# qutech/filter_functions

Hardware: AMD Instinct MI355X
Metric: filter-function elements/sec (n_seg*n_omega*n_nops*d^2) at d=4 (higher is better)
Workload: dtype f64

## Files before the change

### filter_functions_amd/csrc/ctrl_pq.hip

```cpp
#include <algorithm>
#include <cstdlib>

#include "ffk_internal.h"
#include "ffk_mfma_util.h"

namespace ffk {
namespace {

constexpr int kPqProducers = 4;
constexpr int kPqSets = 2;
constexpr int kPqConsumers = 16/kPqSets;
constexpr int kPqRing = 8;
#ifndef FFK_PC_SPIN_LIMIT
#define FFK_PC_SPIN_LIMIT (1 << 21)
#endif
constexpr int kPqSpinLimit = FFK_PC_SPIN_LIMIT;

__device__ __forceinline__ void pq_report_fault(int* fault, int code) {
    if (fault != nullptr && (threadIdx.x & 63) == 0)
        __hip_atomic_store(fault, code, __ATOMIC_RELAXED, __HIP_MEMORY_SCOPE_SYSTEM);
}

typedef double double2_t __attribute__((ext_vector_type(2)));
typedef double double4_t __attribute__((ext_vector_type(4)));
typedef double double8_t __attribute__((ext_vector_type(8)));
typedef int int4_t __attribute__((ext_vector_type(4)));
typedef __attribute__((address_space(3))) int lds_int_t;

template <int NC>
struct PqConsumer;
#include "ctrl_pq_consumer.inc"

constexpr int kPqQ = 0, kPqPsi = 1024, kPqW = 1152;
constexpr int kPqRow = seg_stride(4);
__host__ __device__ constexpr int pq_tile_doubles(int nc) { return kPqW + nc*128 + 32; }
__host__ __device__ constexpr int pq_lds_bytes_for(int nc) {
    return (kPqRing*pq_tile_doubles(nc) + kPqProducers*kPqRow)*8 + 3*kPqRing*4;
}

__device__ __forceinline__ int lds_peek(const int* flag) {
    return __builtin_amdgcn_readfirstlane(*(const volatile lds_int_t*)(flag));
}

template <int NC, bool PRE>
__global__ __launch_bounds__((kPqProducers + kPqConsumers)*64, 3) void ctrl_accumulate_pq_kernel(
    const double* __restrict__ omega, int W, const double* __restrict__ segtab,
    const cplx* __restrict__ ops, int G, int A, int chunk_len, cplx* __restrict__ Ypart,
    const cplx* __restrict__ wfold, int alpha_base, int alpha_end, int* __restrict__ fault_word) {
    constexpr int D = 4, DD = 16, S = kPqRow, TILE = pq_tile_doubles(NC);
    constexpr int TOP = kPqW + NC*128;
    static_assert(PqConsumer<NC>::kTileBytes == TILE*8, "tools/gen_pq_consumer.py and pq_tile_doubles() disagree");
    extern __shared__ __attribute__((aligned(16))) unsigned char lds_raw[];
    double* ring = reinterpret_cast<double*>(lds_raw);
    double* rows = ring + kPqRing*TILE;
    int* ready = reinterpret_cast<int*>(rows + kPqProducers*S);
    int* done = ready + kPqRing;

    const int lane = threadIdx.x & 63;
    const int wave = __builtin_amdgcn_readfirstlane(threadIdx.x >> 6);
    const int alpha0 = alpha_base + blockIdx.y*NC;
    const int n_alpha = min(NC, alpha_end - alpha0);
    const int g0 = blockIdx.z*chunk_len;
    const int g1 = min(G, g0 + chunk_len);
    const int n_it = max(0, g1 - g0);
    int spin_limit = kPqSpinLimit;

    if (threadIdx.x < 3*kPqRing) *(volatile lds_int_t*)(ready + threadIdx.x) = 0;
    __syncthreads();

    if (wave < kPqProducers) {
        __builtin_amdgcn_s_setprio(0);
        const int iw = blockIdx.x*64 + lane;
        double om = omega[iw < W ? iw : W - 1];
        asm volatile("" : "+v"(om));
        const int n_ops = (1 + n_alpha)*DD;
        double* row = rows + wave*S;
        struct Staged {
            cplx o;
            double r0, r1;
        };
        auto request = [&](int it) __attribute__((always_inline)) -> Staged {
            const int g = g0 + it;
            const cplx* src = ops + static_cast<size_t>(g)*(1 + A)*DD;
            const double* st = segtab + static_cast<size_t>(g)*S;
            Staged t;
            if constexpr (PRE) {
                t.o = cplx{0.0, 0.0};
                t.r0 = st[lane];
                t.r1 = st[64 + (lane & (S - 64 - 1))];
            } else {
                t.o = lane < n_ops ? src[lane < DD ? lane : lane + alpha0*DD] : cplx{0.0, 0.0};
                t.r0 = st[lane];
                t.r1 = lane < S - 64 ? st[64 + lane] : 0.0;
            }
            return t;
        };
        auto wait_slot = [&](int slot, int gen) __attribute__((always_inline)) {
            if (gen > 0) {
                int spin = 0;
                for (; spin < spin_limit; ++spin) {
                    if (lds_peek(done + slot) >= gen*kPqConsumers) break;
                    __builtin_amdgcn_s_sleep(2);
                }
                if (spin == spin_limit && spin_limit != 0) {
                    pq_report_fault(fault_word, kFaultPcProducerWait);
                    spin_limit = 0;
                }
                asm volatile("" ::: "memory");
            }
        };
        Staged cur = {};
        if (wave < n_it) cur = request(wave);
        for (int it = wave; it < n_it; it += kPqProducers) {
            const int slot = it & (kPqRing - 1);
            const int gen = it/kPqRing;
            double* buf = ring + slot*TILE;
            row[lane] = cur.r0;
            if (lane < S - 64) row[64 + lane] = cur.r1;
            const cplx o = cur.o;
            if constexpr (PRE) {
                wait_slot(slot, gen);
                const size_t gw = (static_cast<size_t>(g0 + it)*A + alpha0)*64;
#pragma unroll
                for (int a = 0; a < NC; ++a)
                    if (a < n_alpha) lds_dma16(wfold + gw + a*64 + lane, buf + kPqW + a*128);
                if (lane < DD) lds_dma16(ops + static_cast<size_t>(g0 + it)*(1 + A)*DD + lane, buf + TOP);
            }
            if (it + kPqProducers < n_it) cur = request(it + kPqProducers);
            const double* st = row;
            const double2_t sbcb = *reinterpret_cast<const double2_t*>(st + seg_rec(lane >> 2) + 1);
            const double2_t head = *reinterpret_cast<const double2_t*>(st);
            const double sb = sbcb.x, cb = sbcb.y;
            const double dtg = head.x;
            cplx ph;
            sincos_pi<false>(om*head.y, &ph.im, &ph.re);
            double sa, ca;
            sincos_pi<false>(0.5*(om*dtg), &sa, &ca);
            const PhasedFrequency pf = phased_frequency(om, dtg, ph, sa, ca);
            double q[DD];
            auto batch = [&](int e0, int e1) __attribute__((always_inline)) {
                double4_t rec[DD];
#pragma unroll
                for (int e = 0; e < DD; ++e) {
                    if (e < e0 || e >= e1 || (e != 0 && e/D == e%D)) continue;
                    rec[e] = *reinterpret_cast<const double4_t*>(st + seg_rec(e));
                }
                asm volatile("" ::: "memory");
                double xmin = pf.thr;
#pragma unroll
                for (int e = 0; e < DD; ++e) {
                    if (e < e0 || e >= e1 || (e != 0 && e/D == e%D)) continue;
                    const double x = om + rec[e].x;
                    q[e] = fma(pf.sa2, rec[e].z, pf.ca2*rec[e].y)*rcp_fast(x);
                    asm("v_min_f64 %0, |%1|, %0" : "+v"(xmin) : "v"(x));
                }
                if (xmin < pf.thr) {
#pragma unroll
                    for (int e = 0; e < DD; ++e) {
                        if (e < e0 || e >= e1 || (e != 0 && e/D == e%D)) continue;
                        if (fabs(om + rec[e].x) < pf.thr) q[e] = phased_q(pf, rec[e].x, rec[e].y, rec[e].z);
                    }
                }
            };
            batch(0, 8);
            batch(8, 16);
            q[5] = q[0];
            q[10] = q[0];
            q[15] = q[0];
            if constexpr (!PRE) wait_slot(slot, gen);
#pragma unroll
            for (int h = 0; h < 2; ++h)
#pragma unroll
                for (int m = 0; m < D; ++m) {
                    const double2_t v = {q[m*D + 2*h], q[m*D + 2*h + 1]};
                    *reinterpret_cast<double2_t*>(buf + kPqQ + h*512 + lane*8 + (((m ^ (lane >> 2)) & 3) << 1)) = v;
                }
            {
                const double2_t v = {pf.pr, pf.pi};
                *reinterpret_cast<double2_t*>(buf + kPqPsi + lane*2) = v;
            }
            if constexpr (!PRE) {
                const int src_t = lane & (DD - 1);
                const cplx tv = {__shfl(o.re, src_t, 64), __shfl(o.im, src_t, 64)};
                const cplx et = cmul(cplx{cb, sb}, tv);
                const int wslot = ((lane >> 2) & 3)*16 + (lane >> 4)*4 + (lane & 3);
#pragma unroll
                for (int a = 0; a < NC; ++a) {
                    const int src_b = DD + a*DD + (lane >> 2);
                    const cplx bv = {__shfl(o.re, src_b, 64), __shfl(o.im, src_b, 64)};
                    const cplx w = cmul(bv, et);
                    const double2_t v = {w.re, w.im};
                    *reinterpret_cast<double2_t*>(buf + kPqW + a*128 + wslot*2) = v;
                }
            }
            if constexpr (PRE) {
                if (it + kPqProducers < n_it) asm volatile("s_waitcnt vmcnt(2)" ::: "memory");
                else lds_dma_wait();
            } else if (lane < DD) {
                const double2_t v = {o.re, o.im};
                *reinterpret_cast<double2_t*>(buf + TOP + lane*2) = v;
            }
            asm volatile("s_waitcnt lgkmcnt(0)" ::: "memory");
#ifdef FFK_PC_FAULT_INJECT
            if (it < 2*kPqProducers)
#endif
            if (lane == 0) *(volatile lds_int_t*)(ready + slot) = it + 1;
        }
        return;
    }

    const int octant = wave - kPqProducers;
    const int m = lane >> 4, f = (lane >> 2) & 3, j = lane & 3;
    const int mj = m*4 + j;
    const int wf = octant*4*kPqSets + f;
    const int o_w = kPqW + mj*2;
    const int o_p = kPqPsi + wf*2;
    const int o_q0 = kPqQ + wf*8 + ((m ^ ((kPqSets*octant) & 3)) << 1);
    const int o_q1 = (o_q0 ^ 2) + 32;
    double P[6*NC];
#pragma unroll
    for (int k = 0; k < 6*NC; ++k) P[k] = 0.0;
    if (n_it > 0) {
        int spin = 0;
        for (; spin < spin_limit; ++spin) {
            if (lds_peek(ready) >= 1) break;
            __builtin_amdgcn_s_sleep(1);
        }
        if (spin == spin_limit) {
            pq_report_fault(fault_word, kFaultPcConsumerWait);
            spin_limit = 0;
        }
        asm volatile("" ::: "memory");
        const unsigned ring_b = static_cast<unsigned>(reinterpret_cast<uintptr_t>(ring));
        const unsigned flags_b = static_cast<unsigned>(reinterpret_cast<uintptr_t>(ready));
        const int fault_code = PqConsumer<NC>::run(ring_b + o_w*8, ring_b + o_q0*8, ring_b + o_q1*8, ring_b + o_p*8, n_it,
                                                   spin_limit, flags_b, octant, P);
        if (fault_code != 0) pq_report_fault(fault_word, fault_code);
    }
#pragma unroll
    for (int a = 0; a < NC; ++a) {
        const int alpha = alpha0 + a;
        if (alpha >= alpha_end) break;
        cplx* out = Ypart + ((static_cast<size_t>(blockIdx.z)*A + alpha)*DD + mj)*W;
#pragma unroll
        for (int s = 0; s < kPqSets; ++s) {
            const int iw = blockIdx.x*64 + wf + s*4;
            const double p1 = P[3*(kPqSets*a + s)], p2 = P[3*(kPqSets*a + s) + 1], p3 = P[3*(kPqSets*a + s) + 2];
            if (iw < W) out[iw] = cplx{p1 - p2, p3 - (p1 + p2)};
        }
    }
}

template <int NC, bool PRE>
hipError_t launch_pq_as(const double* omega, int W, const double* segtab, const cplx* ops, int G, int A,
                        int chunks, int chunk_len, cplx* Ypart, const cplx* wfold, int alpha_base, int alpha_end,
                        int* fault_word, hipStream_t stream) {
    const int lds = pq_lds_bytes_for(NC);
    auto kern = ctrl_accumulate_pq_kernel<NC, PRE>;
    hipError_t err = hipFuncSetAttribute(reinterpret_cast<const void*>(kern),
                                         hipFuncAttributeMaxDynamicSharedMemorySize, lds);
    if (err != hipSuccess) return err;
    const int n = alpha_end - alpha_base;
    const dim3 grid((W + 63)/64, (n + NC - 1)/NC, chunks);
    hipLaunchKernelGGL(kern, grid, dim3((kPqProducers + kPqConsumers)*64), lds, stream, omega, W, segtab,
                       ops, G, A, chunk_len, Ypart, wfold, alpha_base, alpha_end, fault_word);
    return hipGetLastError();
}

template <int NC>
hipError_t launch_pq(const double* omega, int W, const double* segtab, const cplx* ops, int G, int A,
                     int chunks, int chunk_len, cplx* Ypart, const cplx* wfold, int alpha_base, int alpha_end,
                     int* fault_word, hipStream_t stream) {
    return wfold != nullptr ? launch_pq_as<NC, true>(omega, W, segtab, ops, G, A, chunks, chunk_len, Ypart, wfold,
                                                     alpha_base, alpha_end, fault_word, stream)
                            : launch_pq_as<NC, false>(omega, W, segtab, ops, G, A, chunks, chunk_len, Ypart, nullptr,
                                                      alpha_base, alpha_end, fault_word, stream);
}

}

int pq_accumulate_lds_bytes(int nc) { return pq_lds_bytes_for(nc); }
int pq_accumulate_waves(int) { return kPqProducers + kPqConsumers; }
bool pq_accumulate_supported(int d, int A) { return d == 4 && A >= 1; }

PqGroups pq_accumulate_groups(int A) {
    if (A <= 0) return {0, 0, 0};
    if (A == 1) return {0, 0, 1};
    switch (A % 3) {
        case 0: return {A/3, 0, 0};
        case 1: return {(A - 4)/3, 2, 0};
        default: return {(A - 2)/3, 1, 0};
// ... 29 lines not shown
```

### filter_functions_amd/csrc/ffk_math.h

```cpp
#pragma once

#include <hip/hip_runtime.h>

#include <cmath>

#define FFK_HD __host__ __device__ __forceinline__

namespace ffk {

struct cplx {
    double re, im;
};

FFK_HD cplx cmul(cplx a, cplx b) {
    return {fma(a.re, b.re, -(a.im*b.im)), fma(a.re, b.im, a.im*b.re)};
}
FFK_HD void cmac(cplx& acc, cplx a, cplx b) {
    acc.re = fma(a.re, b.re, acc.re);
    acc.re = fma(-a.im, b.im, acc.re);
    acc.im = fma(a.re, b.im, acc.im);
    acc.im = fma(a.im, b.re, acc.im);
}
FFK_HD void cmac_conj(cplx& acc, cplx a, cplx b) {
    acc.re = fma(a.re, b.re, acc.re);
    acc.re = fma(a.im, b.im, acc.re);
    acc.im = fma(a.re, b.im, acc.im);
    acc.im = fma(-a.im, b.re, acc.im);
}

template <unsigned long long BITS>
FFK_HD double pinned_bits() {
#if defined(__HIP_DEVICE_COMPILE__)
    unsigned lo, hi;
    asm volatile("v_mov_b32 %0, %1" : "=v"(lo) : "n"(static_cast<unsigned>(BITS & 0xffffffffull)));
    asm volatile("v_mov_b32 %0, %1" : "=v"(hi) : "n"(static_cast<unsigned>(BITS >> 32)));
    return __hiloint2double(static_cast<int>(hi), static_cast<int>(lo));
#else
    return __builtin_bit_cast(double, BITS);
#endif
}
#define FFK_PIN(c) (PIN ? pinned_bits<__builtin_bit_cast(unsigned long long, static_cast<double>(c))>() : (c))

template <bool PIN = false>
FFK_HD void sincos_reduced(double r, double* s, double* c) {
    const double z = r*r;
    double ps = fma(z, FFK_PIN(1.58969099521155010221e-10), FFK_PIN(-2.50507602534068634195e-08));
    ps = fma(z, ps, FFK_PIN(2.75573137070700676789e-06));
    ps = fma(z, ps, FFK_PIN(-1.98412698298579493134e-04));
    ps = fma(z, ps, FFK_PIN(8.33333333332248946124e-03));
    ps = fma(z, ps, FFK_PIN(-1.66666666666666324348e-01));
    *s = fma(r*z, ps, r);
    double pc = fma(z, FFK_PIN(-1.13596475577881948265e-11), FFK_PIN(2.08757232129817482790e-09));
    pc = fma(z, pc, FFK_PIN(-2.75573143513906633035e-07));
    pc = fma(z, pc, FFK_PIN(2.48015872894767294178e-05));
    pc = fma(z, pc, FFK_PIN(-1.38888888888741095749e-03));
    pc = fma(z, pc, FFK_PIN(4.16666666666666019037e-02));
    const double hz = 0.5*z;
    const double w = 1.0 - hz;
    *c = w + (((1.0 - w) - hz) + z*z*pc);
}

template <bool PIN = false>
FFK_HD void sincos_small(double r, double* s, double* c) {
    const double z = r*r;
    double ps = fma(z, FFK_PIN(2.75573137070700676789e-06), FFK_PIN(-1.98412698298579493134e-04));
    ps = fma(z, ps, FFK_PIN(8.33333333332248946124e-03));
    ps = fma(z, ps, FFK_PIN(-1.66666666666666324348e-01));
    *s = fma(r*z, ps, r);
    double pc = fma(z, FFK_PIN(2.48015872894767294178e-05), FFK_PIN(-1.38888888888741095749e-03));
    pc = fma(z, pc, FFK_PIN(4.16666666666666019037e-02));
    const double hz = 0.5*z;
    const double w = 1.0 - hz;
    *c = w + (((1.0 - w) - hz) + z*z*pc);
}

FFK_HD unsigned low_word(double t) {
#if defined(__HIP_DEVICE_COMPILE__)
    return static_cast<unsigned>(__double2loint(t));
#else
    unsigned long long bits;
    __builtin_memcpy(&bits, &t, sizeof bits);
    return static_cast<unsigned>(bits);
#endif
}

template <bool PIN = false>
FFK_HD void sincos_pi(double x, double* s, double* c) {
    const double kMagic = FFK_PIN(6755399441055744.0);
    const double t = fma(x, FFK_PIN(6.36619772367581382433e-01), kMagic);
    const unsigned q = low_word(t);
    const double k = t - kMagic;
    double r = fma(-k, FFK_PIN(1.57079632679489655800e+00), x);
    r = fma(-k, FFK_PIN(6.12323399573676603587e-17), r);
    r = fma(-k, FFK_PIN(-1.49738490485916983294e-33), r);
    double sr, cr;
    sincos_reduced<PIN>(r, &sr, &cr);
    const double s0 = (q & 1u) ? cr : sr;
    const double c0 = (q & 1u) ? sr : cr;
    *s = (q & 2u) ? -s0 : s0;
    *c = ((q + 1u) & 2u) ? -c0 : c0;
}

#undef FFK_PIN

FFK_HD double rcp(double x) {
#if defined(__HIP_DEVICE_COMPILE__)
    double y = __builtin_amdgcn_rcp(x);
    double e = fma(-x, y, 1.0);
    y = fma(y, e, y);
    e = fma(-x, y, 1.0);
    y = fma(y, e, y);
    return y;
#else
    return 1.0/x;
#endif
}

FFK_HD double rcp_fast(double x) {
#if defined(__HIP_DEVICE_COMPILE__)
    double y = __builtin_amdgcn_rcp(x);
    const double e = fma(-x, y, 1.0);
    return fma(y, e, y);
#else
    return 1.0/x;
#endif
}

FFK_HD double rsqrt(double x) {
#if defined(__HIP_DEVICE_COMPILE__)
    double y = __builtin_amdgcn_rsq(x);
    double e = fma(-x*y, y, 1.0);
    y = fma(y, 0.5*e, y);
    e = fma(-x*y, y, 1.0);
    y = fma(y, 0.5*e, y);
    return y;
#else
    return 1.0/sqrt(x);
#endif
}

FFK_HD cplx first_order_integral(double omega, double dE, double dt) {
    const double x = omega + dE;
    const double y = x*dt;
    double s, c;
    sincos_pi(0.5*y, &s, &c);
    const double q = 2.0*s*rcp(x);
    cplx out = {q*c, q*s};
    if (x == 0.0) {
        out.re = dt;
        out.im = 0.0;
    }
    return out;
}

FFK_HD cplx first_order_integral_aa(double omega, double dE, double dt, double sa, double ca,
                                    double sb, double cb) {
    const double x = omega + dE;
    const double h = 0.5*(x*dt);
    double s = fma(sa, cb, ca*sb);
    double c = fma(ca, cb, -(sa*sb));
    if (fabs(h) < 0.03125) sincos_small<true>(h, &s, &c);
    const double q = 2.0*s*rcp_fast(x);
    cplx out = {q*c, q*s};
    if (x == 0.0) {
        out.re = dt;
        out.im = 0.0;
    }
    return out;
}

struct PhasedFrequency {
    double om, dt, thr;
    double pr, pi;
    double sa2, ca2;
};
FFK_HD PhasedFrequency phased_frequency(double om, double dt, cplx ph, double sa, double ca) {
    PhasedFrequency f;
    f.om = om;
    f.dt = dt;
    f.thr = dt > 0.0 ? 0.0625*rcp(dt) : __builtin_huge_val();
    f.pr = fma(ph.re, ca, -(ph.im*sa));
    f.pi = fma(ph.re, sa, ph.im*ca);
    f.sa2 = sa + sa;
    f.ca2 = ca + ca;
    return f;
}
FFK_HD double phased_q(const PhasedFrequency& f, double dE, double sb, double cb) {
    const double x = f.om + dE;
    double q;
    if (fabs(x) < f.thr) {
        double s, c;
        sincos_small<true>(0.5*(x*f.dt), &s, &c);
        q = x == 0.0 ? f.dt : 2.0*s*rcp_fast(x);
    } else {
        q = fma(f.sa2, cb, f.ca2*sb)*rcp_fast(x);
    }
    return q;
}
FFK_HD cplx phased_integral_aa(const PhasedFrequency& f, double dE, double sb, double cb) {
    const double er = fma(f.pr, cb, -(f.pi*sb));
    const double ei = fma(f.pr, sb, f.pi*cb);
    const double q = phased_q(f, dE, sb, cb);
    return {q*er, q*ei};
}

FFK_HD cplx cexp(double x) {
    cplx out;
    sincos_pi(x, &out.im, &out.re);
    return out;
}

}
```

### filter_functions_amd/csrc/post.hip

```cpp
#include <algorithm>

#include <cstdlib>

#include "ffk_internal.h"

namespace ffk {
namespace {

__global__ void reduce_chunks_kernel(const cplx* __restrict__ Ypart, int chunks, size_t slab,
                                     cplx* __restrict__ Bt) {
    const size_t e = static_cast<size_t>(blockIdx.x)*blockDim.x + threadIdx.x;
    if (e >= slab) return;
    cplx acc = Ypart[e];
    for (int c = 1; c < chunks; ++c) {
        const cplx v = Ypart[static_cast<size_t>(c)*slab + e];
        acc.re += v.re;
        acc.im += v.im;
    }
    Bt[e] = acc;
}

__global__ __launch_bounds__(64) void basis_compact_kernel(const cplx* __restrict__ basis, int d,
                                                           int* __restrict__ nnz,
                                                           int* __restrict__ rows,
// ... 198 lines not shown
    const int a0 = ba*TB, b0 = bb*TB;
    cplx acc[TB][TB];
#pragma unroll
    for (int i = 0; i < TB; ++i)
#pragma unroll
        for (int j = 0; j < TB; ++j) acc[i][j] = {0.0, 0.0};
    for (int k = 0; k < N; ++k) {
        cplx ra[TB], rb[TB];
#pragma unroll
        for (int i = 0; i < TB; ++i) {
            const int a = min(a0 + i, A - 1), b = min(b0 + i, A - 1);
            ra[i] = R[(static_cast<size_t>(a)*N + k)*W + w];
            rb[i] = R[(static_cast<size_t>(b)*N + k)*W + w];
        }
#pragma unroll
        for (int i = 0; i < TB; ++i)
#pragma unroll
            for (int j = 0; j < TB; ++j) cmac_conj(acc[i][j], ra[i], rb[j]);
    }
#pragma unroll
    for (int i = 0; i < TB; ++i)
#pragma unroll
        for (int j = 0; j < TB; ++j) {
            const int a = a0 + i, b = b0 + j;
            if (a >= A || b >= A || a > b) continue;
            cplx v = acc[i][j];
            if (a == b) v.im = 0.0;
            F[(static_cast<size_t>(a)*A + b)*W + w] = v;
            if (a != b) F[(static_cast<size_t>(b)*A + a)*W + w] = {v.re, -v.im};
        }
    }
}

template <int TB, int NT>
__global__ __launch_bounds__(NT*64) void ff_fidelity_lds_kernel(const cplx* __restrict__ R, int A, int N, int W,
                                                             int kc, cplx* __restrict__ F) {
    extern __shared__ __attribute__((aligned(16))) unsigned char ffl_raw[];
    cplx* buf = reinterpret_cast<cplx*>(ffl_raw);
    const int tid = threadIdx.x, lane = tid & 63;
    const int wave = __builtin_amdgcn_readfirstlane(tid >> 6);
    const int nwaves = blockDim.x >> 6;
    const int nb = (A + TB - 1)/TB;
    int ba = 0, rem = wave;
    while (rem >= nb - ba) {
        rem -= nb - ba;
        ++ba;
    }
    const int bb = ba + rem;
    const int a0 = ba*TB, b0 = bb*TB;
    const int w0 = blockIdx.x*64;
    const int w = w0 + lane;
    const int wc = min(w, W - 1);
    const int rows = kc*A;
    constexpr int kMaxRows = 12;
    const cplx* src[kMaxRows];
    int dst[kMaxRows];
#pragma unroll
    for (int r = 0; r < kMaxRows; ++r) {
        const int row = min(wave + r*nwaves, rows - 1);
        src[r] = R + (static_cast<size_t>(row % A)*N + row / A)*W + wc;
        dst[r] = row*64 + lane;
    }
    cplx acc[TB][TB];
#pragma unroll
    for (int i = 0; i < TB; ++i)
#pragma unroll
        for (int j = 0; j < TB; ++j) acc[i][j] = {0.0, 0.0};
#pragma unroll
    for (int r = 0; r < kMaxRows; ++r) buf[dst[r]] = src[r][0];
    __syncthreads();
    int b = 0;
    for (int k0 = 0; k0 < N; k0 += kc) {
        cplx staged[kMaxRows];
        const size_t knext = static_cast<size_t>(min(k0 + kc, N - kc < 0 ? 0 : N - kc))*W;
#pragma unroll
        for (int r = 0; r < kMaxRows; ++r) staged[r] = src[r][knext];
        const int kn = min(kc, N - k0);
        for (int kk = 0; kk < kn; ++kk) {
            const cplx* rowp = buf + (static_cast<size_t>(b)*rows + kk*A)*64 + lane;
            cplx ra[TB], rb[TB];
#pragma unroll
            for (int i = 0; i < TB; ++i) {
                ra[i] = rowp[min(a0 + i, A - 1)*64];
                rb[i] = rowp[min(b0 + i, A - 1)*64];
            }
#pragma unroll
            for (int i = 0; i < TB; ++i)
#pragma unroll
                for (int j = 0; j < TB; ++j) cmac_conj(acc[i][j], ra[i], rb[j]);
        }
#pragma unroll
        for (int r = 0; r < kMaxRows; ++r) buf[static_cast<size_t>(b ^ 1)*rows*64 + dst[r]] = staged[r];
        __syncthreads();
        b ^= 1;
    }
    if (w >= W) return;
#pragma unroll
    for (int i = 0; i < TB; ++i)
#pragma unroll
        for (int j = 0; j < TB; ++j) {
            const int a = a0 + i, bq = b0 + j;
            if (a >= A || bq >= A || a > bq) continue;
            cplx v = acc[i][j];
            if (a == bq) v.im = 0.0;
            F[(static_cast<size_t>(a)*A + bq)*W + w] = v;
            if (a != bq) F[(static_cast<size_t>(bq)*A + a)*W + w] = {v.re, -v.im};
        }
}

__global__ __launch_bounds__(128) void ff_weighted_kernel(const cplx* __restrict__ R, int A, int N,
                                                          int W, const cplx* __restrict__ M,
                                                          double scale, cplx* __restrict__ F) {
    const int w = blockIdx.x*blockDim.x + threadIdx.x;
    if (w >= W) return;
    for (long long pair = blockIdx.y; pair < static_cast<long long>(A)*A; pair += gridDim.y) {
        const int a = static_cast<int>(pair / A), b = static_cast<int>(pair % A);
        const cplx* ra = R + static_cast<size_t>(a)*N*W + w;
        const cplx* rb = R + static_cast<size_t>(b)*N*W + w;
        cplx acc = {0.0, 0.0};
        for (int k = 0; k < N; ++k) {
            cplx u = {0.0, 0.0};
            for (int l = 0; l < N; ++l) cmac(u, M[k*N + l], rb[static_cast<size_t>(l)*W]);
            cmac_conj(acc, ra[static_cast<size_t>(k)*W], u);
        }
        F[(static_cast<size_t>(a)*A + b)*W + w] = {scale*acc.re, scale*acc.im};
    }
}

__global__ void ff_generalized_kernel(const cplx* __restrict__ R, int A, int N, int W,
                                      cplx* __restrict__ F) {
    const int w = blockIdx.x*blockDim.x + threadIdx.x;
    if (w >= W) return;
    for (long long ab = blockIdx.z; ab < static_cast<long long>(A)*A; ab += gridDim.z) {
        const int a = static_cast<int>(ab / A), b = static_cast<int>(ab % A);
        for (long long kl = blockIdx.y; kl < static_cast<long long>(N)*N; kl += gridDim.y) {
            const int k = static_cast<int>(kl / N), l = static_cast<int>(kl % N);
            const cplx x = R[(static_cast<size_t>(a)*N + k)*W + w];
            const cplx y = R[(static_cast<size_t>(b)*N + l)*W + w];
            const double rr = x.re*y.re;
            const double ii = x.im*y.im;
            const double ri = x.re*y.im;
            const double ir = x.im*y.re;
            cplx v;
            v.re = rr + ii;
            v.im = ri - ir;
            F[((((static_cast<size_t>(a)*A + b)*N + k)*N + l))*W + w] = v;
        }
    }
}

constexpr int kInfidSlots = 1024, kInfidThreads = 256;
constexpr int kInfidPer = kInfidSlots/kInfidThreads;

template <int J0, int JN, typename LoadF, typename LoadS>
__device__ __forceinline__ void infid_batch(int base, int W, const double* __restrict__ omega, LoadF Fat, LoadS Sat,
                                            double (&acc)[kInfidPer], double* red = nullptr) {
    const int lane = threadIdx.x & 63;
    cplx f[kInfidPer], sp[kInfidPer];
    double om[kInfidPer];
#pragma unroll
    for (int j = J0; j < J0 + JN; ++j) {
        const int w = base + static_cast<int>(threadIdx.x) + kInfidThreads*j;
        const int wc = w < W ? w : W - 1;
        f[j] = Fat(wc);
        sp[j] = Sat(wc);
        om[j] = omega[wc];
    }
#pragma unroll
    for (int j = J0; j < J0 + JN; ++j) {
        const int w = base + static_cast<int>(threadIdx.x) + kInfidThreads*j;
        const double i0 = f[j].re*sp[j].re - f[j].im*sp[j].im;
        double i1 = __shfl_down(i0, 1, 64), o1 = __shfl_down(om[j], 1, 64);
        if (lane == 63 && w + 1 < W) {
            const cplx f1 = Fat(w + 1), s1 = Sat(w + 1);
            i1 = f1.re*s1.re - f1.im*s1.im;
            o1 = omega[w + 1];
        }
        if (w < W - 1) {
            if (red != nullptr) red[threadIdx.x + kInfidThreads*j] += (i1 + i0)*(o1 - om[j]);
            else acc[j] += (i1 + i0)*(o1 - om[j]);
        }
    }
}

template <bool FROM_REGISTERS = true>
__device__ __forceinline__ void infid_finish(double* red, const double (&acc)[kInfidPer], int d, double* out) {
    static_assert(kInfidPer == 4 && kInfidThreads == 256, "the tree below is written for 4 slots per thread, 4 wavefronts");
    double sl[kInfidPer];
#pragma unroll
    for (int j = 0; j < kInfidPer; ++j) sl[j] = FROM_REGISTERS ? acc[j] : red[threadIdx.x + kInfidThreads*j];
    double x = (sl[0] + sl[2]) + (sl[1] + sl[3]);
    __syncthreads();
    red[threadIdx.x] = x;
    __syncthreads();
    if (threadIdx.x < 128) red[threadIdx.x] = x = x + red[threadIdx.x + 128];
    __syncthreads();
    if (threadIdx.x < 64) {
        x = x + red[threadIdx.x + 64];
#pragma unroll
        for (int off = 32; off > 0; off >>= 1) x = x + __shfl_down(x, off, 64);
        if (threadIdx.x == 0) *out = (x/2.0)/(2.0*3.141592653589793*d);
    }
}

template <bool SHARDED>
__device__ __forceinline__ void infid_element(const cplx* __restrict__ F, int A, int W,
                                              const cplx* __restrict__ S, int s_ndim,
                                              const double* __restrict__ omega,
                                              const int32_t* __restrict__ idx, int n_idx,
                                              int d, int shard_width,
                                              double* __restrict__ infid, const int p) {
    __shared__ double red[kInfidSlots];
    __builtin_amdgcn_s_setprio(3);
    int ia, ib;
    const cplx* Sp;
    if (s_ndim == 3) {
        ia = idx[p / n_idx];
        ib = idx[p % n_idx];
        Sp = S + static_cast<size_t>(p)*W;
    } else {
        ia = ib = idx[p];
        Sp = S + (s_ndim == 2 ? static_cast<size_t>(p)*W : 0);
    }
    const cplx* Fp = F + (static_cast<size_t>(ia)*A + ib)*(SHARDED ? shard_width : W);
    auto Fat = [&](int w) -> cplx {
        if (SHARDED) {
            const int r = w / shard_width, wl = w - r*shard_width;
            return Fp[static_cast<size_t>(r)*A*A*shard_width + wl];
        }
        return Fp[w];
    };
    auto Sat = [&](int w) -> cplx { return Sp[w]; };
    double acc[kInfidPer];
#pragma unroll
    for (int j = 0; j < kInfidPer; ++j) red[threadIdx.x + kInfidThreads*j] = 0.0;
    for (int base = 0; base < W - 1; base += kInfidSlots) {
        infid_batch<0, kInfidPer>(base, W, omega, Fat, Sat, acc, red);
        asm volatile("" ::: "memory");
    }
    infid_finish<false>(red, acc, d, infid + p);
}

template <bool SHARDED>
__global__ __launch_bounds__(kInfidThreads) void infid_kernel(const cplx* __restrict__ F, int A, int W,
                                                              const cplx* __restrict__ S, int s_ndim,
                                                              const double* __restrict__ omega,
                                                              const int32_t* __restrict__ idx, int n_idx,
                                                              int d, int shard_width,
                                                              double* __restrict__ infid) {
    infid_element<SHARDED>(F, A, W, S, s_ndim, omega, idx, n_idx, d, shard_width, infid, blockIdx.x);
}

__global__ __launch_bounds__(kInfidThreads) void infid_pulses_kernel(const cplx* __restrict__ F, int A, int W,
                                                                     const cplx* __restrict__ S, int s_ndim,
                                                                     const double* __restrict__ omega,
                                                                     const int32_t* __restrict__ idx, int n_idx,
                                                                     int d, int nout, double* __restrict__ infid) {
    const size_t q = blockIdx.y;
    infid_element<false>(F + q*A*A*W, A, W, S, s_ndim, omega, idx, n_idx, d, 0, infid + q*nout, blockIdx.x);
}

constexpr int kInfidStage = 4096;
__global__ __launch_bounds__(kInfidThreads) void infid_host_spectrum_kernel(
    const cplx* __restrict__ F, int A, int W, const cplx* __restrict__ S, int s_ndim,
    const double* __restrict__ omega, const int32_t* __restrict__ idx, int n_idx, int d,
    double* __restrict__ infid) {
    __shared__ double red[kInfidSlots];
    extern __shared__ __attribute__((aligned(16))) unsigned char stage_raw[];
    cplx* sl = reinterpret_cast<cplx*>(stage_raw);
    const int p = blockIdx.x;
    int ia, ib;
    const cplx* Sp;
    if (s_ndim == 3) {
        ia = idx[p / n_idx];
        ib = idx[p % n_idx];
        Sp = S + static_cast<size_t>(p)*W;
    } else {
        ia = ib = idx[p];
        Sp = S + (s_ndim == 2 ? static_cast<size_t>(p)*W : 0);
    }
    const cplx* Fp = F + (static_cast<size_t>(ia)*A + ib)*W;
    constexpr int kLoads = kInfidStage/kInfidThreads + 1;
    double acc[kInfidPer];
#pragma unroll
    for (int j = 0; j < kInfidPer; ++j) acc[j] = 0.0;
    for (int s0 = 0; s0 < W - 1; s0 += kInfidStage) {
        const int n = min(kInfidStage + 1, W - s0);
        cplx v[kLoads];
#pragma unroll
        for (int k = 0; k < kLoads; ++k) {
            const int i = threadIdx.x + kInfidThreads*k;
            v[k] = i < n ? Sp[s0 + i] : cplx{0.0, 0.0};
        }
#pragma unroll
        for (int k = 0; k < kLoads; ++k) {
            const int i = threadIdx.x + kInfidThreads*k;
            if (i < n) sl[i] = v[k];
        }
        __syncthreads();
        auto Fat = [&](int w) -> cplx { return Fp[w]; };
        auto Sat = [&](int w) -> cplx { return sl[w - s0]; };
        const int bend = min(W - 1, s0 + kInfidStage);
        for (int base = s0; base < bend; base += kInfidSlots) infid_batch<0, kInfidPer>(base, W, omega, Fat, Sat, acc);
        __syncthreads();
    }
    infid_finish(red, acc, d, infid + p);
}

}

hipError_t launch_reduce_chunks(const cplx* Ypart, int chunks, size_t slab, cplx* Bt,
                                hipStream_t stream) {
    const int block = 256;
    hipLaunchKernelGGL(reduce_chunks_kernel, dim3(static_cast<unsigned>((slab + block - 1)/block)),
                       dim3(block), 0, stream, Ypart, chunks, slab, Bt);
    return hipGetLastError();
}

size_t expand_workspace_bytes(int N, int d) {
    const size_t dd = static_cast<size_t>(d)*d;
    return align_up(sizeof(int)*N) + align_up(sizeof(int)*N*dd) + align_up(sizeof(cplx)*N*dd);
}

namespace {
struct CompactWs {
    int* nnz;
    int* rows;
    cplx* vals;
};
CompactWs slice_compact_ws(void* ws, int N, int d) {
    const size_t dd = static_cast<size_t>(d)*d;
    unsigned char* p = static_cast<unsigned char*>(ws);
    CompactWs out;
    out.nnz = reinterpret_cast<int*>(p);
    p += align_up(sizeof(int)*N);
    out.rows = reinterpret_cast<int*>(p);
    p += align_up(sizeof(int)*N*dd);
    out.vals = reinterpret_cast<cplx*>(p);
    return out;
}
}

hipError_t launch_reduce_and_compact(const cplx* Ypart, int chunks, size_t slab, cplx* Bt,
                                     const cplx* basis, int N, int d, void* ws, hipStream_t stream) {
    const CompactWs c = slice_compact_ws(ws, N, d);
    const int block = 256;
    const int nred = static_cast<int>((slab + block - 1)/block);
    hipLaunchKernelGGL(reduce_compact_kernel, dim3(nred + N), dim3(block), 0, stream, Ypart, chunks,
                       slab, Bt, nred, basis, d, c.nnz, c.rows, c.vals);
    return hipGetLastError();
}

void expand_workspace_slices(void* ws, int N, int d, int** nnz, int** rows, cplx** vals) {
    const CompactWs cw = slice_compact_ws(ws, N, d);
    *nnz = cw.nnz;
    *rows = cw.rows;
    *vals = cw.vals;
}

__global__ __launch_bounds__(64) void expand_chunks_kernel(const cplx* __restrict__ Ypart, int chunks,
                                                           size_t slab, const int* __restrict__ nnz,
                                                           const int* __restrict__ rows,
                                                           const cplx* __restrict__ vals, int N,
                                                           int dd, int W, cplx* __restrict__ R) {
    const int w = blockIdx.x*64 + threadIdx.x;
    const int a = blockIdx.y, k = blockIdx.z;
    if (w >= W) return;
    const cplx* b = Ypart + static_cast<size_t>(a)*dd*W + w;
    const int n = nnz[k];
    const int* rk = rows + static_cast<size_t>(k)*dd;
    const cplx* vk = vals + static_cast<size_t>(k)*dd;
    auto summed = [&](int e) {
        cplx acc = b[static_cast<size_t>(e)*W];
        for (int z = 1; z < chunks; ++z) {
            const cplx v = b[z*slab + static_cast<size_t>(e)*W];
            acc.re += v.re;
            acc.im += v.im;
        }
        return acc;
    };
    cplx acc0 = {0.0, 0.0}, acc1 = {0.0, 0.0};
    int q = 0;
    for (; q + 1 < n; q += 2) {
        cmac(acc0, vk[q], summed(rk[q]));
        cmac(acc1, vk[q + 1], summed(rk[q + 1]));
    }
    if (q < n) cmac(acc0, vk[q], summed(rk[q]));
    R[(static_cast<size_t>(a)*N + k)*W + w] = {acc0.re + acc1.re, acc0.im + acc1.im};
}

__device__ __forceinline__ void expand_ff_tile(const cplx* __restrict__ Ypart, int chunks, size_t slab,
                                               const int* __restrict__ nnz, const int* __restrict__ rows,
                                               const cplx* __restrict__ vals, int N, int dd, int W, int A,
                                               int kt, cplx* __restrict__ R, cplx* __restrict__ F) {
    extern __shared__ __attribute__((aligned(16))) unsigned char lds_raw[];
    cplx* rl = reinterpret_cast<cplx*>(lds_raw);
    __builtin_amdgcn_s_setprio(3);
    cplx* ys = rl + static_cast<size_t>(A)*N*16;
    const int wl = threadIdx.x & 15;
    const int kl = (threadIdx.x >> 4) % kt, al = (threadIdx.x >> 4) / kt;
    const int at = (blockDim.x >> 4) / kt;
    const int w = blockIdx.x*16 + wl;
    const int wc = w < W ? w : W - 1;
    for (int idx = threadIdx.x >> 4; idx < A*dd; idx += blockDim.x >> 4) {
        const cplx* b = Ypart + static_cast<size_t>(idx)*W + wc;
        cplx acc = b[0];
        for (int z = 1; z < chunks; ++z) {
            const cplx v = b[z*slab];
            acc.re += v.re;
            acc.im += v.im;
        }
        ys[static_cast<size_t>(idx)*16 + wl] = acc;
    }
    __syncthreads();
    for (int a = al; a < A; a += at) {
        const cplx* ya = ys + static_cast<size_t>(a)*dd*16 + wl;
        for (int k = kl; k < N; k += kt) {
            const int n = nnz[k];
            const int* rk = rows + static_cast<size_t>(k)*dd;
            const cplx* vk = vals + static_cast<size_t>(k)*dd;
            auto summed = [&](int e) { return ya[e*16]; };
            cplx acc0 = {0.0, 0.0}, acc1 = {0.0, 0.0};
            int q = 0;
            for (; q + 1 < n; q += 2) {
                cmac(acc0, vk[q], summed(rk[q]));
                cmac(acc1, vk[q + 1], summed(rk[q + 1]));
            }
            if (q < n) cmac(acc0, vk[q], summed(rk[q]));
            const cplx r = {acc0.re + acc1.re, acc0.im + acc1.im};
            rl[(static_cast<size_t>(a)*N + k)*16 + wl] = r;
            if (w < W) R[(static_cast<size_t>(a)*N + k)*W + w] = r;
        }
    }
    __syncthreads();
    if (w >= W) return;
    const int npairs = A*(A + 1)/2;
    const int lanes = blockDim.x >> 4;
    for (int p = threadIdx.x >> 4; p < npairs; p += lanes) {
        int a = 0, rem = p;
        while (rem >= A - a) {
            rem -= A - a;
            ++a;
        }
        const int b = a + rem;
        const cplx* ra = rl + static_cast<size_t>(a)*N*16 + wl;
        const cplx* rb = rl + static_cast<size_t>(b)*N*16 + wl;
        cplx acc = {0.0, 0.0};
        for (int k = 0; k < N; ++k) cmac_conj(acc, ra[k*16], rb[k*16]);
        if (a == b) acc.im = 0.0;
        F[(static_cast<size_t>(a)*A + b)*W + w] = acc;
        if (a != b) F[(static_cast<size_t>(b)*A + a)*W + w] = {acc.re, -acc.im};
    }
}

__global__ __launch_bounds__(256) void expand_ff_kernel(const cplx* __restrict__ Ypart, int chunks,
                                                         size_t slab, const int* __restrict__ nnz,
// ... 265 lines not shown
```

### filter_functions_amd/csrc/prep.hip

```cpp
#include "ffk_internal.h"

namespace ffk {
namespace {

template <int D>
__device__ void prologue_segment(const cplx (*V)[D], cplx (*Q)[D], cplx (*T)[D], cplx (*BV)[D],
                                 int g, int lane, const double* __restrict__ eigvals,
                                 const cplx* __restrict__ n_opers,
                                 const double* __restrict__ n_coeffs,
                                 const double* __restrict__ dt, const double* __restrict__ t, int G,
                                 int A, double* __restrict__ segtab, cplx* __restrict__ Tc,
                                 cplx* __restrict__ ops, cplx* __restrict__ n_opers_transformed,
                                 cplx* __restrict__ eigvecs_propagated, bool with_noise_ops = true,
                                 cplx* __restrict__ wfold = nullptr) {
    constexpr int S = seg_stride(D);
    double* st = segtab + static_cast<size_t>(g)*S;
    if (lane == 0) {
        st[0] = dt[g];
        st[1] = t[g];
    }
    cplx eb = {1.0, 0.0};
    for (int e = lane; e < D*D; e += 64) {
        const double dE = eigvals[static_cast<size_t>(g)*D + e / D] - eigvals[static_cast<size_t>(g)*D + e % D];
        double sb, cb;
        sincos_pi(0.5*(dE*dt[g]), &sb, &cb);
        st[seg_rec(e)] = dE;
        st[seg_rec(e) + 1] = sb;
        st[seg_rec(e) + 2] = cb;
        st[seg_rec(e) + 3] = 0.0;
        eb = {cb, sb};
    }
    if (lane < 2) st[2 + lane] = 0.0;
    for (int e = 4 + 4*D*D + lane; e < S; e += 64) st[e] = 0.0;

    for (int e = lane; e < D*D; e += 64) {
        const int m = e / D, j = e % D;
        cplx acc = {0.0, 0.0};
#pragma unroll
        for (int k = 0; k < D; ++k) cmac_conj(acc, V[k][m], Q[k][j]);
        T[m][j] = acc;
        Tc[static_cast<size_t>(g)*D*D + e] = {acc.re, -acc.im};
        ops[static_cast<size_t>(g)*(1 + A)*D*D + e] = acc;
        if (eigvecs_propagated)
            eigvecs_propagated[static_cast<size_t>(g)*D*D + j*D + m] = {acc.re, -acc.im};
    }
    __syncthreads();

    if (!with_noise_ops) return;
    const bool fold = D == 4 && wfold != nullptr;
    if (fold) {
        if (lane < D*D) Q[lane / D][lane % D] = eb;
        __syncthreads();
    }
    for (int a = 0; a < A; ++a) {
        const cplx* B = n_opers + static_cast<size_t>(a)*D*D;
        const double s = n_coeffs ? n_coeffs[static_cast<size_t>(a)*G + g] : 1.0;
        for (int e = lane; e < D*D; e += 64) {
            const int i = e / D, n = e % D;
            cplx acc = {0.0, 0.0};
#pragma unroll
            for (int k = 0; k < D; ++k) cmac(acc, B[i*D + k], V[k][n]);
            BV[i][n] = acc;
        }
        __syncthreads();
        cplx bbar = {0.0, 0.0};
        for (int e = lane; e < D*D; e += 64) {
            const int m = e / D, n = e % D;
            cplx acc = {0.0, 0.0};
#pragma unroll
            for (int k = 0; k < D; ++k) cmac_conj(acc, V[k][m], BV[k][n]);
            acc.re *= s;
            acc.im *= s;
            ops[(static_cast<size_t>(g)*(1 + A) + 1 + a)*D*D + e] = acc;
            if (n_opers_transformed)
                n_opers_transformed[(static_cast<size_t>(a)*G + g)*D*D + e] = acc;
            if (fold) bbar = acc;
        }
        __syncthreads();
        if (fold) {
            if (lane < D*D) BV[lane / D][lane % D] = bbar;
            __syncthreads();
            if constexpr (D == 4) {
                const int m = lane >> 4, n = (lane >> 2) & 3, j = lane & 3;
                const cplx et = cmul(Q[m][n], T[n][j]);
                const cplx w = cmul(BV[m][n], et);
                wfold[(static_cast<size_t>(g)*A + a)*64 + n*16 + m*4 + j] = w;
            }
            __syncthreads();
        }
    }
}

template <int D>
__global__ __launch_bounds__(64) void prologue_kernel(
    const double* __restrict__ eigvals, const cplx* __restrict__ eigvecs,
    const cplx* __restrict__ propagators, const cplx* __restrict__ n_opers,
    const double* __restrict__ n_coeffs, const double* __restrict__ dt,
    const double* __restrict__ t, int G, int A, double* __restrict__ segtab,
    cplx* __restrict__ Tc, cplx* __restrict__ ops, cplx* __restrict__ n_opers_transformed,
    cplx* __restrict__ eigvecs_propagated, bool with_noise_ops, cplx* __restrict__ wfold) {
    __shared__ cplx V[D][D];
    __shared__ cplx Q[D][D];
    __shared__ cplx T[D][D];
    __shared__ cplx BV[D][D];
    const int g = blockIdx.x;
    const int lane = threadIdx.x;
    for (int e = lane; e < D*D; e += 64) {
        V[e / D][e % D] = eigvecs[static_cast<size_t>(g)*D*D + e];
        Q[e / D][e % D] = propagators[static_cast<size_t>(g)*D*D + e];
    }
    __syncthreads();
    prologue_segment<D>(V, Q, T, BV, g, lane, eigvals, n_opers, n_coeffs, dt, t, G, A, segtab, Tc,
                        ops, n_opers_transformed, eigvecs_propagated, with_noise_ops, wfold);
}

template <int D>
__global__ __launch_bounds__(64) void noise_ops_kernel(const cplx* __restrict__ eigvecs,
                                                       const cplx* __restrict__ n_opers,
                                                       const double* __restrict__ n_coeffs, int G,
                                                       int A, cplx* __restrict__ ops,
                                                       cplx* __restrict__ n_opers_transformed) {
    __shared__ cplx V[D][D];
    __shared__ cplx BV[D][D];
    __builtin_amdgcn_s_setprio(3);
    const int g = blockIdx.x, a = blockIdx.y, lane = threadIdx.x;
    for (int e = lane; e < D*D; e += 64) V[e / D][e % D] = eigvecs[static_cast<size_t>(g)*D*D + e];
    __syncthreads();
    const cplx* B = n_opers + static_cast<size_t>(a)*D*D;
    const double s = n_coeffs ? n_coeffs[static_cast<size_t>(a)*G + g] : 1.0;
    for (int e = lane; e < D*D; e += 64) {
        const int i = e / D, n = e % D;
        cplx acc = {0.0, 0.0};
#pragma unroll
        for (int k = 0; k < D; ++k) cmac(acc, B[i*D + k], V[k][n]);
        BV[i][n] = acc;
    }
    __syncthreads();
    for (int e = lane; e < D*D; e += 64) {
        const int m = e / D, n = e % D;
        cplx acc = {0.0, 0.0};
#pragma unroll
        for (int k = 0; k < D; ++k) cmac_conj(acc, V[k][m], BV[k][n]);
        acc.re *= s;
        acc.im *= s;
        ops[(static_cast<size_t>(g)*(1 + A) + 1 + a)*D*D + e] = acc;
        if (n_opers_transformed)
            n_opers_transformed[(static_cast<size_t>(a)*G + g)*D*D + e] = acc;
    }
}

constexpr int kNoiseOpsKernelMinD = 12;
inline bool split_noise_ops(int d, int A) { return d >= kNoiseOpsKernelMinD && A >= 2 && A <= 65535; }

template <int D>
__device__ __forceinline__ void apply_prologue_segment(
    const cplx* __restrict__ Qloc, const cplx* __restrict__ totals, int G, int L,
    cplx* __restrict__ Qout, const double* __restrict__ eigvals, const cplx* __restrict__ eigvecs,
    const cplx* __restrict__ n_opers, const double* __restrict__ n_coeffs,
    const double* __restrict__ dt, const double* __restrict__ t, int A,
    double* __restrict__ segtab, cplx* __restrict__ Tc, cplx* __restrict__ ops,
    bool with_noise_ops, cplx* __restrict__ wfold, const int g) {
    __builtin_amdgcn_s_setprio(3);
    __shared__ cplx E[2][D][D];
    __shared__ cplx M[D][D];
    __shared__ cplx V[D][D];
    __shared__ cplx Q[D][D];
    __shared__ cplx T[D][D];
    __shared__ cplx BV[D][D];
    constexpr int kBatch = 16;
    constexpr bool kTree = D <= 8;
    extern __shared__ __attribute__((aligned(16))) unsigned char tot_raw[];
    cplx (*tot)[D][D] = reinterpret_cast<cplx (*)[D][D]>(tot_raw);
    const int lane = threadIdx.x;
    const int c = g / L;
    for (int e = lane; e < D*D; e += 64) E[0][e / D][e % D] = {(e / D == e % D) ? 1.0 : 0.0, 0.0};
    int b = 0;
    if constexpr (kTree) {
        constexpr int DD = D*D, PER = 64/DD;
        for (int e = lane; e < c*DD; e += 64) (&tot[0][0][0])[e] = totals[e];
        __syncthreads();
        int n = c;
        while (n > 1) {
            const int pairs = n >> 1;
            for (int j0 = 0; j0 < pairs; j0 += PER) {
                const int jj = j0 + lane/DD, e = lane % DD, i = e / D, k = e % D;
// ... 341 lines not shown
```

Before: 916.4 billion.

## Precompute per-segment resonance threshold and prefetch wave-edge infidelity neighbours

The resonance threshold 0.0625/dt is now computed once per segment in the prologue and stored in the unused header slot of the segment table. The control kernel reads it with a wider header load instead of evaluating a Newton-refined reciprocal for every omega. Separately, the infidelity batch now loads the neighbour element just past each wave's edge up front, once per slot, instead of doing a divergent load on lane 63 only. In the main path those values are forced into scalar registers. The cost is a wider header load, extra registers, and inline asm scalar constraints that could raise register pressure or fail to compile on some paths.

```diff
diff --git a/filter_functions_amd/csrc/ctrl_pq.hip b/filter_functions_amd/csrc/ctrl_pq.hip
--- a/filter_functions_amd/csrc/ctrl_pq.hip
+++ b/filter_functions_amd/csrc/ctrl_pq.hip
@@ -129,14 +129,14 @@
             if (it + kPqProducers < n_it) cur = request(it + kPqProducers);
             const double* st = row;
             const double2_t sbcb = *reinterpret_cast<const double2_t*>(st + seg_rec(lane >> 2) + 1);
-            const double2_t head = *reinterpret_cast<const double2_t*>(st);
+            const double4_t head = *reinterpret_cast<const double4_t*>(st);
             const double sb = sbcb.x, cb = sbcb.y;
             const double dtg = head.x;
             cplx ph;
             sincos_pi<false>(om*head.y, &ph.im, &ph.re);
             double sa, ca;
             sincos_pi<false>(0.5*(om*dtg), &sa, &ca);
-            const PhasedFrequency pf = phased_frequency(om, dtg, ph, sa, ca);
+            const PhasedFrequency pf = phased_frequency(om, dtg, head.z, ph, sa, ca);
             double q[DD];
             auto batch = [&](int e0, int e1) __attribute__((always_inline)) {
                 double4_t rec[DD];
diff --git a/filter_functions_amd/csrc/ffk_math.h b/filter_functions_amd/csrc/ffk_math.h
--- a/filter_functions_amd/csrc/ffk_math.h
+++ b/filter_functions_amd/csrc/ffk_math.h
@@ -174,16 +174,20 @@
     double pr, pi;
     double sa2, ca2;
 };
-FFK_HD PhasedFrequency phased_frequency(double om, double dt, cplx ph, double sa, double ca) {
+FFK_HD double resonance_threshold(double dt) { return dt > 0.0 ? 0.0625*rcp(dt) : __builtin_huge_val(); }
+FFK_HD PhasedFrequency phased_frequency(double om, double dt, double thr, cplx ph, double sa, double ca) {
     PhasedFrequency f;
     f.om = om;
     f.dt = dt;
-    f.thr = dt > 0.0 ? 0.0625*rcp(dt) : __builtin_huge_val();
+    f.thr = thr;
     f.pr = fma(ph.re, ca, -(ph.im*sa));
     f.pi = fma(ph.re, sa, ph.im*ca);
     f.sa2 = sa + sa;
     f.ca2 = ca + ca;
     return f;
+}
+FFK_HD PhasedFrequency phased_frequency(double om, double dt, cplx ph, double sa, double ca) {
+    return phased_frequency(om, dt, resonance_threshold(dt), ph, sa, ca);
 }
 FFK_HD double phased_q(const PhasedFrequency& f, double dE, double sb, double cb) {
     const double x = f.om + dE;
diff --git a/filter_functions_amd/csrc/post.hip b/filter_functions_amd/csrc/post.hip
--- a/filter_functions_amd/csrc/post.hip
+++ b/filter_functions_amd/csrc/post.hip
@@ -374,12 +374,21 @@
 constexpr int kInfidSlots = 1024, kInfidThreads = 256;
 constexpr int kInfidPer = kInfidSlots/kInfidThreads;
 
-template <int J0, int JN, typename LoadF, typename LoadS>
+template <int J0, int JN, bool EDGE_SCALAR, typename LoadF, typename LoadS>
 __device__ __forceinline__ void infid_batch(int base, int W, const double* __restrict__ omega, LoadF Fat, LoadS Sat,
                                             double (&acc)[kInfidPer], double* red = nullptr) {
     const int lane = threadIdx.x & 63;
-    cplx f[kInfidPer], sp[kInfidPer];
-    double om[kInfidPer];
+    const int behind = __builtin_amdgcn_readfirstlane(static_cast<int>(threadIdx.x) | 63) + 1;
+    cplx f[kInfidPer], sp[kInfidPer], fe[kInfidPer], se[kInfidPer];
+    double om[kInfidPer], oe[kInfidPer];
+#pragma unroll
+    for (int j = J0; j < J0 + JN; ++j) {
+        const int we = base + behind + kInfidThreads*j;
+        const int wec = we < W ? we : W - 1;
+        fe[j] = Fat(wec);
+        se[j] = Sat(wec);
+        oe[j] = omega[wec];
+    }
 #pragma unroll
     for (int j = J0; j < J0 + JN; ++j) {
         const int w = base + static_cast<int>(threadIdx.x) + kInfidThreads*j;
@@ -388,15 +397,25 @@
         sp[j] = Sat(wc);
         om[j] = omega[wc];
     }
+    if constexpr (EDGE_SCALAR) {
+        static_assert(JN == 4 || JN == 2, "one statement for all slots of the batch: one wait, before any of the lanes' loads is");
+        if constexpr (JN == 4)
+            asm volatile("" : "+s"(fe[J0].re), "+s"(fe[J0].im), "+s"(se[J0].re), "+s"(se[J0].im), "+s"(oe[J0]),
+                              "+s"(fe[J0 + 1].re), "+s"(fe[J0 + 1].im), "+s"(se[J0 + 1].re), "+s"(se[J0 + 1].im), "+s"(oe[J0 + 1]),
+                              "+s"(fe[J0 + 2].re), "+s"(fe[J0 + 2].im), "+s"(se[J0 + 2].re), "+s"(se[J0 + 2].im), "+s"(oe[J0 + 2]),
+                              "+s"(fe[J0 + 3].re), "+s"(fe[J0 + 3].im), "+s"(se[J0 + 3].re), "+s"(se[J0 + 3].im), "+s"(oe[J0 + 3]));
+        else
+            asm volatile("" : "+s"(fe[J0].re), "+s"(fe[J0].im), "+s"(se[J0].re), "+s"(se[J0].im), "+s"(oe[J0]),
+                              "+s"(fe[J0 + 1].re), "+s"(fe[J0 + 1].im), "+s"(se[J0 + 1].re), "+s"(se[J0 + 1].im), "+s"(oe[J0 + 1]));
+    }
 #pragma unroll
     for (int j = J0; j < J0 + JN; ++j) {
         const int w = base + static_cast<int>(threadIdx.x) + kInfidThreads*j;
         const double i0 = f[j].re*sp[j].re - f[j].im*sp[j].im;
         double i1 = __shfl_down(i0, 1, 64), o1 = __shfl_down(om[j], 1, 64);
-        if (lane == 63 && w + 1 < W) {
-            const cplx f1 = Fat(w + 1), s1 = Sat(w + 1);
-            i1 = f1.re*s1.re - f1.im*s1.im;
-            o1 = omega[w + 1];
+        if (lane == 63) {
+            i1 = fe[j].re*se[j].re - fe[j].im*se[j].im;
+            o1 = oe[j];
         }
         if (w < W - 1) {
             if (red != nullptr) red[threadIdx.x + kInfidThreads*j] += (i1 + i0)*(o1 - om[j]);
@@ -457,7 +476,7 @@
 #pragma unroll
     for (int j = 0; j < kInfidPer; ++j) red[threadIdx.x + kInfidThreads*j] = 0.0;
     for (int base = 0; base < W - 1; base += kInfidSlots) {
-        infid_batch<0, kInfidPer>(base, W, omega, Fat, Sat, acc, red);
+        infid_batch<0, kInfidPer, true>(base, W, omega, Fat, Sat, acc, red);
         asm volatile("" ::: "memory");
     }
     infid_finish<false>(red, acc, d, infid + p);
@@ -523,7 +542,7 @@
         auto Fat = [&](int w) -> cplx { return Fp[w]; };
         auto Sat = [&](int w) -> cplx { return sl[w - s0]; };
         const int bend = min(W - 1, s0 + kInfidStage);
-        for (int base = s0; base < bend; base += kInfidSlots) infid_batch<0, kInfidPer>(base, W, omega, Fat, Sat, acc);
+        for (int base = s0; base < bend; base += kInfidSlots) infid_batch<0, kInfidPer, false>(base, W, omega, Fat, Sat, acc);
         __syncthreads();
     }
     infid_finish(red, acc, d, infid + p);
diff --git a/filter_functions_amd/csrc/prep.hip b/filter_functions_amd/csrc/prep.hip
--- a/filter_functions_amd/csrc/prep.hip
+++ b/filter_functions_amd/csrc/prep.hip
@@ -18,6 +18,8 @@
     if (lane == 0) {
         st[0] = dt[g];
         st[1] = t[g];
+        st[2] = resonance_threshold(dt[g]);
+        st[3] = 0.0;
     }
     cplx eb = {1.0, 0.0};
     for (int e = lane; e < D*D; e += 64) {
@@ -30,7 +32,6 @@
         st[seg_rec(e) + 3] = 0.0;
         eb = {cb, sb};
     }
-    if (lane < 2) st[2 + lane] = 0.0;
     for (int e = 4 + 4*D*D + lane; e < S; e += 64) st[e] = 0.0;
 
     for (int e = lane; e < D*D; e += 64) {
```

Measured after the change: 924.8 billion (median of 6 runs). About the same (+0.9%).
